# evroon/mav-detection

Measured on NVIDIA B200. Metric: 1080p frame-pairs/sec (flow+FoE+mask), higher is better.
Workload: dtype f32

## Files before the change

mav_detection_b200/csrc/farneback.cu:

```cuda
#include <math.h>

#include "common.cuh"

namespace mavd {

__device__ __forceinline__ int reflect101(int i, int n) {
    while (i < 0 || i >= n) {
        if (n == 1) return 0;
        i = (i < 0) ? -i : 2 * (n - 1) - i;
    }
    return i;
}

__device__ __forceinline__ int clampi(int v, int lo, int hi) { return v < lo ? lo : (v > hi ? hi : v); }

struct PyrLevel {
    int w, h, pitch, taps;
    const int* xbase; const float* xtab;
    const float* xtabT;
    int staged;
    const int* ybase; const float* ytab;
    float* tmp; float* img;
    size_t tmp_stride, img_stride;
    int row0;
// ... 747 lines not shown
            for (int idx = tid; idx < RH * RW; idx += 256) {
                int rr = idx / RW, cc = idx - rr * RW;
                int gy = clampi(y0 - m + rr, 0, h - 1);
                int gx = clampi(x0 - hx + cc, 0, w - 1);
                raw[idx] = __ldg(src + (size_t)gy * pitch + gx);
            }
        }
        __syncthreads();
        const int ncols = IT_TX + 2 * m;
        if (!GAUSS) {
            for (int task = tid; task < ncols * 4; task += 256) {
                int cc = task % ncols + (hx - m), seg = task / ncols;
                const float* col = raw + (seg * 8) * RW + cc;
                float s = 0.f;
                for (int j = 0; j <= 2 * m; ++j) s += col[j * RW];
                float* dst = vs + (seg * 8) * RW + cc;
                dst[0] = s;
#pragma unroll
                for (int o = 1; o < 8; ++o) {
                    s += col[(o + 2 * m) * RW] - col[(o - 1) * RW];
                    dst[o * RW] = s;
                }
            }
        } else {
            for (int task = tid; task < ncols * IT_TY; task += 256) {
                int cc = task % ncols + (hx - m), r = task / ncols;
                const float* col = raw + r * RW + cc;
                float s = __fmul_rn(col[m * RW], __ldg(a.gk));
                for (int i = 1; i <= m; ++i) s = __fmaf_rn(col[(m - i) * RW] + col[(m + i) * RW], __ldg(a.gk + i), s);
                vs[r * RW + cc] = s;
            }
        }
        __syncthreads();
        float* Sc = S + c * (IT_TY * IT_TX);
        if (hx == 8 && m >= 5) {
            for (int task = tid; task < IT_TY * (IT_TX / 4); task += 256) {
                int q = task & 15, r = task >> 4;
                const float4* pv = reinterpret_cast<const float4*>(vs + r * RW + 4 * q);
                float u[20];
#pragma unroll
                for (int j = 0; j < 5; ++j) {
                    float4 v = pv[j];
                    u[4 * j] = v.x; u[4 * j + 1] = v.y; u[4 * j + 2] = v.z; u[4 * j + 3] = v.w;
                }
                float o[4];
                if (!GAUSS) {
                    switch (m) {
                        case 5: hsum_box<5>(u, o); break;
                        case 6: hsum_box<6>(u, o); break;
                        case 7: hsum_box<7>(u, o); break;
                        default: hsum_box<8>(u, o); break;
                    }
                } else {
                    switch (m) {
                        case 5: hsum_gauss<5>(u, a.gk, o); break;
                        case 6: hsum_gauss<6>(u, a.gk, o); break;
                        case 7: hsum_gauss<7>(u, a.gk, o); break;
                        default: hsum_gauss<8>(u, a.gk, o); break;
                    }
                }
                *reinterpret_cast<float4*>(Sc + r * IT_TX + 4 * q) = make_float4(o[0], o[1], o[2], o[3]);
            }
        } else {
            for (int idx = tid; idx < IT_TY * IT_TX; idx += 256) {
                int cx = idx & 63, r = idx >> 6;
                const float* row = vs + r * RW + hx + cx;
                float s;
                if (!GAUSS) {
                    s = 0.f;
                    for (int j = -m; j <= m; ++j) s += row[j];
                } else {
                    s = __fmul_rn(row[0], __ldg(a.gk));
                    for (int i = 1; i <= m; ++i) s = __fmaf_rn(row[-i] + row[i], __ldg(a.gk + i), s);
                }
                Sc[idx] = s;
            }
        }
    }
    __syncthreads();

    const float* R0 = a.R + (size_t)(p * a.pair_stride) * 5 * plane;
    const float* R1 = R0 + 5 * plane;
    float* Mout = LAST ? nullptr : a.Mout + (size_t)p * 5 * plane;
#pragma unroll 2
    for (int j = 0; j < (IT_TX * IT_TY) / 256; ++j) {
        const int idx = j * 256 + tid;
        const int cx = idx & 63, r = idx >> 6;
        const int x = x0 + cx, y = y0 + r;
        if (x >= w || y >= h) continue;
        const float g11 = S[idx] * a.scale, g12 = S[IT_TX * IT_TY + idx] * a.scale,
                    g22 = S[2 * IT_TX * IT_TY + idx] * a.scale, h1 = S[3 * IT_TX * IT_TY + idx] * a.scale,
                    h2 = S[4 * IT_TX * IT_TY + idx] * a.scale;
        const float idet = 1.f / (g11 * g22 - g12 * g12 + 1e-3f);
        const float fx = (g11 * h2 - g12 * h1) * idet;
        const float fy = (g22 * h1 - g12 * h2) * idet;
        if (a.flow) a.flow[(size_t)p * a.flow_stride + (size_t)y * a.flow_pitch + x] = make_float2(fx, fy);
        if (!LAST) update_matrices_px(x, y, w, h, pitch, plane, fx, fy, load_r0_px(R0, (size_t)y * pitch + x, plane), R1, Mout);
    }
}

__device__ __forceinline__ uint32_t smem_u32(const void* p) { return (uint32_t)__cvta_generic_to_shared(p); }

__device__ __forceinline__ void mbar_init(uint64_t* bar, uint32_t count) {
    asm volatile("mbarrier.init.shared::cta.b64 [%0], %1;" ::"r"(smem_u32(bar)), "r"(count));
    asm volatile("fence.mbarrier_init.release.cluster;" ::: "memory");
}
__device__ __forceinline__ void mbar_expect_tx(uint64_t* bar, uint32_t bytes) {
    asm volatile("mbarrier.arrive.expect_tx.shared::cta.b64 _, [%0], %1;" ::"r"(smem_u32(bar)), "r"(bytes) : "memory");
}
__device__ __forceinline__ void mbar_wait(uint64_t* bar, uint32_t parity) {
    asm volatile(
        "{\n"
        ".reg .pred P1;\n"
        "LAB_WAIT:\n"
        "mbarrier.try_wait.parity.shared::cta.b64 P1, [%0], %1;\n"
        "@P1 bra DONE;\n"
        "bra LAB_WAIT;\n"
        "DONE:\n"
        "}" ::"r"(smem_u32(bar)), "r"(parity) : "memory");
}
__device__ __forceinline__ void tma_load_3d(void* dst, const CUtensorMap* map, int c0, int c1, int c2, uint64_t* bar) {
    asm volatile(
        "cp.async.bulk.tensor.3d.shared::cluster.global.mbarrier::complete_tx::bytes [%0], [%1, {%2, %3, %4}], [%5];"
        ::"r"(smem_u32(dst)), "l"(map), "r"(c0), "r"(c1), "r"(c2), "r"(smem_u32(bar)) : "memory");
}

__device__ __forceinline__ void tma_prefetch_3d(const CUtensorMap* map, int c0, int c1, int c2) {
    asm volatile("cp.async.bulk.prefetch.tensor.3d.L2.global.tile [%0, {%1, %2, %3}];"
                 ::"l"(map), "r"(c0), "r"(c1), "r"(c2) : "memory");
}

constexpr int PE_BW = 96;

template <bool U8, int N_>
__global__ void __launch_bounds__(256, 4) polyexp_tma_kernel(const __grid_constant__ CUtensorMap tmap, int w, int h,
                                                         int pitch, PolyConst pc, float* __restrict__ R, size_t plane) {
    pdl_entry();
    __shared__ __align__(128) float raw[(PE_TY + 2 * PE_H) * PE_RW];
    __shared__ __align__(128) float t[3][PE_TY * PE_RW];
    __shared__ __align__(8) uint64_t bar;
    const int tid = threadIdx.x;
    const int x0 = blockIdx.x * PE_TX, y0 = blockIdx.y * PE_TY;
    const int n = N_ > 0 ? N_ : pc.n;
    const int rows = PE_TY + 2 * n;
    uint8_t* bytes = reinterpret_cast<uint8_t*>(&t[0][0]);
    float* raw0 = raw;
    if (tid == 0) {
        mbar_init(&bar, 1);
        if (U8) {
            mbar_expect_tx(&bar, (uint32_t)((rows + 2) * PE_BW));
            tma_load_3d(bytes, &tmap, x0 - 16, y0 - n - 1, blockIdx.z, &bar);
        } else {
            mbar_expect_tx(&bar, (uint32_t)(rows * PE_RW * sizeof(float)));
            tma_load_3d(raw0, &tmap, x0 - PE_H, y0 - n, blockIdx.z, &bar);
        }
    }
    const bool interior = (x0 - PE_H - 1 >= 0) && (x0 + PE_TX + PE_H + 1 <= w) && (y0 - n - 1 >= 0) &&
                          (y0 + PE_TY + n + 1 <= h);
    __syncthreads();
    mbar_wait(&bar, 0);
    if (U8) {
        if (!interior) {
            for (int rr = tid; rr < rows + 2; rr += 256) {
                uint8_t* row = bytes + rr * PE_BW;
                const int bl = -1 - (x0 - 16), br = w - (x0 - 16);
                if (bl >= 0 && bl + 2 < PE_BW) row[bl] = row[bl + 2];
                if (br >= 2 && br < PE_BW) row[br] = row[br - 2];
            }
            __syncthreads();
            for (int cc = tid; cc < PE_BW; cc += 256) {
                const int bt = -1 - (y0 - n - 1), bb = h - (y0 - n - 1);
                if (bt >= 0 && bt + 2 < rows + 2) bytes[bt * PE_BW + cc] = bytes[(bt + 2) * PE_BW + cc];
                if (bb >= 2 && bb < rows + 2) bytes[bb * PE_BW + cc] = bytes[(bb - 2) * PE_BW + cc];
            }
            __syncthreads();
        }
        const int g = tid % 20, seg = tid / 20;
        const int rps = (rows + 11) / 12;
        const int r0 = seg * rps, r1 = min(rows, r0 + rps);
        if (seg < 12 && r0 < r1) {
            const uint32_t* wp = reinterpret_cast<const uint32_t*>(bytes + r0 * PE_BW + 4 * g + 4);
            float hp[4], hc[4], hn[4];
            blur3_words(wp[0], wp[1], wp[2], hp);
            blur3_words(wp[PE_BW / 4], wp[PE_BW / 4 + 1], wp[PE_BW / 4 + 2], hc);
            for (int i = 0; i < r1 - r0; ++i) {
                const uint32_t* q = wp + (i + 2) * (PE_BW / 4);
                blur3_words(q[0], q[1], q[2], hn);
                float4 v;
                v.x = 0.25f * hp[0] + 0.5f * hc[0] + 0.25f * hn[0];
                v.y = 0.25f * hp[1] + 0.5f * hc[1] + 0.25f * hn[1];
                v.z = 0.25f * hp[2] + 0.5f * hc[2] + 0.25f * hn[2];
                v.w = 0.25f * hp[3] + 0.5f * hc[3] + 0.25f * hn[3];
                *reinterpret_cast<float4*>(&raw0[(r0 + i) * PE_RW + 4 * g]) = v;
#pragma unroll
                for (int k = 0; k < 4; ++k) { hp[k] = hc[k]; hc[k] = hn[k]; }
            }
        }
        __syncthreads();
    }
    if (!interior) {
        const int xlo = max(0, PE_H - x0), xhi = min(PE_RW, w - x0 + PE_H);
        const int ylo = max(0, n - y0), yhi = min(rows, h - y0 + n);
        const int ncol = xlo + (PE_RW - xhi);
        if (ncol > 0) {
            for (int idx = tid; idx < (yhi - ylo) * ncol; idx += 256) {
                const int rr = ylo + idx / ncol, k = idx % ncol;
                float* row = raw0 + rr * PE_RW;
                row[k < xlo ? k : xhi + (k - xlo)] = row[k < xlo ? xlo : xhi - 1];
            }
            __syncthreads();
        }
        const int nrow_out = ylo + (rows - yhi);
        if (nrow_out > 0) {
            for (int idx = tid; idx < nrow_out * (PE_RW / 4); idx += 256) {
                const int k = idx / (PE_RW / 4), q = idx - k * (PE_RW / 4);
                const int rr = k < ylo ? k : yhi + (k - ylo);
                reinterpret_cast<float4*>(raw0 + rr * PE_RW)[q] =
                    reinterpret_cast<const float4*>(raw0 + (k < ylo ? ylo : yhi - 1) * PE_RW)[q];
            }
            __syncthreads();
        }
    }
    polyexp_passes<N_>(raw0 - (PE_H - n) * PE_RW, t, pc, n, tid, x0, y0, h, pitch, R + (size_t)blockIdx.z * 5 * plane, plane);
}


__device__ __forceinline__ R0Px load_r0(const float* __restrict__ R0, unsigned o, unsigned plane) {
    R0Px r;
    r.y = __ldg(R0 + o); r.x = __ldg(R0 + (o + plane)); r.yy = __ldg(R0 + (o + 2 * plane));
    r.xx = __ldg(R0 + (o + 3 * plane)); r.xy = __ldg(R0 + (o + 4 * plane));
    return r;
}

template <int RW, int RH>
__device__ __forceinline__ void update_matrices_box(int x, int y, int w, int h, int pitch, unsigned plane, bool edge, float dx,
                                                    float dy, const R0Px& r0, const float* __restrict__ R1,
                                                    float* __restrict__ Mout, const float* box, int bx, int by) {
    constexpr int CH = RH * RW;
    const unsigned o = (unsigned)(y * pitch + x);
    const float r0y = r0.y, r0x = r0.x, r0yy = r0.yy, r0xx = r0.xx, r0xy = r0.xy;
    float fx = (float)x + dx, fy = (float)y + dy;
    const float flx = floorf(fx), fly = floorf(fy);
    const int x1 = (int)fminf(fmaxf(flx, -2.f), 1.0e6f), y1 = (int)fminf(fmaxf(fly, -2.f), 1.0e6f);
    fx -= flx;
    fy -= fly;
    float r2, r3, r4, r5, r6;
    if ((unsigned)x1 < (unsigned)(w - 1) && (unsigned)y1 < (unsigned)(h - 1)) {
        const float gx = 1.f - fx, gy = 1.f - fy;
        const float a00 = gx * gy, a01 = fx * gy, a10 = gx * fy, a11 = fx * fy;
        const int lx = x1 - bx, ly = y1 - by;
        if ((unsigned)lx < (unsigned)(RW - 1) && (unsigned)ly < (unsigned)(RH - 1)) {
            const float* q = box + ly * RW + lx;
            r2 = a00 * q[0] + a01 * q[1] + a10 * q[RW] + a11 * q[RW + 1];
            r3 = a00 * q[CH] + a01 * q[CH + 1] + a10 * q[CH + RW] + a11 * q[CH + RW + 1];
            r4 = a00 * q[2 * CH] + a01 * q[2 * CH + 1] + a10 * q[2 * CH + RW] + a11 * q[2 * CH + RW + 1];
            r5 = a00 * q[3 * CH] + a01 * q[3 * CH + 1] + a10 * q[3 * CH + RW] + a11 * q[3 * CH + RW + 1];
            r6 = a00 * q[4 * CH] + a01 * q[4 * CH + 1] + a10 * q[4 * CH + RW] + a11 * q[4 * CH + RW + 1];
        } else {
            const unsigned q0 = (unsigned)(y1 * pitch + x1), q1 = q0 + (unsigned)pitch;
            r2 = a00 * __ldg(R1 + q0) + a01 * __ldg(R1 + q0 + 1) + a10 * __ldg(R1 + q1) + a11 * __ldg(R1 + q1 + 1);
            r3 = a00 * __ldg(R1 + (q0 + plane)) + a01 * __ldg(R1 + (q0 + plane) + 1) +
                 a10 * __ldg(R1 + (q1 + plane)) + a11 * __ldg(R1 + (q1 + plane) + 1);
            r4 = a00 * __ldg(R1 + (q0 + 2 * plane)) + a01 * __ldg(R1 + (q0 + 2 * plane) + 1) +
                 a10 * __ldg(R1 + (q1 + 2 * plane)) + a11 * __ldg(R1 + (q1 + 2 * plane) + 1);
            r5 = a00 * __ldg(R1 + (q0 + 3 * plane)) + a01 * __ldg(R1 + (q0 + 3 * plane) + 1) +
                 a10 * __ldg(R1 + (q1 + 3 * plane)) + a11 * __ldg(R1 + (q1 + 3 * plane) + 1);
            r6 = a00 * __ldg(R1 + (q0 + 4 * plane)) + a01 * __ldg(R1 + (q0 + 4 * plane) + 1) +
                 a10 * __ldg(R1 + (q1 + 4 * plane)) + a11 * __ldg(R1 + (q1 + 4 * plane) + 1);
        }
        r4 = (r0yy + r4) * 0.5f;
        r5 = (r0xx + r5) * 0.5f;
        r6 = (r0xy + r6) * 0.25f;
    } else {
        r2 = r3 = 0.f;
        r4 = r0yy;
        r5 = r0xx;
        r6 = r0xy * 0.5f;
    }
    r2 = (r0y - r2) * 0.5f;
    r3 = (r0x - r3) * 0.5f;
    r2 += r4 * dy + r6 * dx;
    r3 += r6 * dy + r5 * dx;
    if (edge && ((unsigned)(x - 5) >= (unsigned)(w - 10) || (unsigned)(y - 5) >= (unsigned)(h - 10))) {
        const float sc = (x < 5 ? border_factor(x) : 1.f) * (x >= w - 5 ? border_factor(w - x - 1) : 1.f) *
                         (y < 5 ? border_factor(y) : 1.f) * (y >= h - 5 ? border_factor(h - y - 1) : 1.f);
        r2 *= sc; r3 *= sc; r4 *= sc; r5 *= sc; r6 *= sc;
    }
    st_global_f32(Mout + o, r4 * r4 + r6 * r6);
    st_global_f32(Mout + (o + plane), (r4 + r5) * r6);
    st_global_f32(Mout + (o + 2 * plane), r5 * r5 + r6 * r6);
    st_global_f32(Mout + (o + 3 * plane), r4 * r2 + r6 * r3);
    st_global_f32(Mout + (o + 4 * plane), r6 * r2 + r5 * r3);
}

template <int M_, bool LAST, int TY, bool GAUSS>
__global__ void __launch_bounds__(256, 3) iter_box_tma_kernel(const __grid_constant__ CUtensorMap tmap,
                                                              const __grid_constant__ CUtensorMap tmapR,
                                                              const __grid_constant__ CUtensorMap tmapRbox, IterArgs a) {
    pdl_entry();
    constexpr int NT = 256;
    constexpr int RW = IT_TX + 16;
    constexpr int RH = TY + 2 * M_;
    constexpr int CH = RH * RW;
    constexpr int NC = IT_TX + 2 * M_;
    constexpr int NW = NT / 32;
    extern __shared__ __align__(128) float box[];
    __shared__ __align__(8) uint64_t bar;
    const int tid = threadIdx.x, lane = tid & 31, warp = tid >> 5;
    const int n_tiles = gridDim.x / a.n_pairs;
    int p, tile;
    if (LAST) {
        p = blockIdx.x / n_tiles;
        tile = blockIdx.x - p * n_tiles;
    } else {
        const int per_group = IT_PAIR_GROUP * n_tiles;
        const int gidx = blockIdx.x / per_group, rem = blockIdx.x - gidx * per_group;
        const int gsize = min(IT_PAIR_GROUP, a.n_pairs - gidx * IT_PAIR_GROUP);
        tile = rem / gsize;
        p = gidx * IT_PAIR_GROUP + (rem - tile * gsize);
    }
    const int x0 = (tile % a.tiles_x) * IT_TX, y0 = (tile / a.tiles_x) * TY;
    const int w = a.w, h = a.h, pitch = a.pitch;
    const int plane = (int)a.plane;
    float gk[M_ + 1];
#pragma unroll
    for (int i = 0; i <= M_; ++i) gk[i] = GAUSS ? __ldg(a.gk + i) : 0.f;
    auto hsum = [&](const float (&u)[20], float (&o)[4]) {
        if (GAUSS) hsum_gauss_reg<M_>(u, gk, o);
        else hsum_box<M_>(u, o);
    };

    if (tid == 0) {
        mbar_init(&bar, 1);
        mbar_expect_tx(&bar, 5 * CH * (uint32_t)sizeof(float));
        tma_load_3d(box, &tmap, x0 - 8, y0 - M_, p * 5, &bar);
        if (!LAST) tma_prefetch_3d(&tmapR, x0 - 8, y0 - 8, p * a.pair_stride * 5);
    }
    const bool interior = (x0 - 8 >= 0) && (x0 + IT_TX + 8 <= w) && (y0 - M_ >= 0) && (y0 + TY + M_ <= h);
    __syncthreads();
    mbar_wait(&bar, 0);

    if (!interior) {
        const int xlo = max(0, 8 - x0), xhi = min(RW, w - x0 + 8);
        const int ylo = max(0, M_ - y0), yhi = min(RH, h - y0 + M_);
        const int ncol = xlo + (RW - xhi), nrow_in = yhi - ylo;
        if (ncol > 0) {
            const int per_plane = nrow_in * ncol;
            for (int idx = tid; idx < 5 * per_plane; idx += NT) {
                const int c = idx / per_plane, rem = idx - c * per_plane;
                const int rr = ylo + rem / ncol, k = rem % ncol;
                const int cc = k < xlo ? k : xhi + (k - xlo);
                float* row = box + c * CH + rr * RW;
                row[cc] = row[k < xlo ? xlo : xhi - 1];
            }
            __syncthreads();
        }
        const int nrow_out = ylo + (RH - yhi);
        if (nrow_out > 0) {
            const int per_plane = nrow_out * (RW / 4);
            for (int idx = tid; idx < 5 * per_plane; idx += NT) {
                const int c = idx / per_plane, rem = idx - c * per_plane;
                const int k = rem / (RW / 4), q = rem - k * (RW / 4);
                const int rr = k < ylo ? k : yhi + (k - ylo);
                float* pl = box + c * CH;
                reinterpret_cast<float4*>(pl + rr * RW)[q] = reinterpret_cast<const float4*>(pl + (k < ylo ? ylo : yhi - 1) * RW)[q];
            }
            __syncthreads();
        }
    }

    for (int t = warp; t < 15; t += NW) {
        const int c = t / 3, col = (t - 3 * c) * 32 + lane;
        if (col < NC) {
            float* q = box + c * CH + (8 - M_) + col;
            float in[RH];
            float s = 0.f;
#pragma unroll
            for (int j = 0; j <= 2 * M_; ++j) {
                in[j] = q[j * RW];
                s += in[j];
            }
            if (GAUSS) {
#pragma unroll
                for (int y = 0; y < TY; ++y) {
                    float g = __fmul_rn(in[y + M_], gk[0]);
#pragma unroll
                    for (int i = 1; i <= M_; ++i) g = __fmaf_rn(in[y + M_ - i] + in[y + M_ + i], gk[i], g);
                    q[y * RW] = g;
                    if (y < TY - 1) in[y + 2 * M_ + 1] = q[(y + 2 * M_ + 1) * RW];
                }
                continue;
            }
#pragma unroll
            for (int y = 0; y < TY; ++y) {
                q[y * RW] = s;
                if (y < TY - 1) {
                    in[y + 2 * M_ + 1] = q[(y + 2 * M_ + 1) * RW];
                    if (((y + 1) & 7) == 0) {
                        s = 0.f;
#pragma unroll
                        for (int j = 0; j <= 2 * M_; ++j) s += in[y + 1 + j];
                    } else {
                        s += in[y + 2 * M_ + 1] - in[y];
                    }
                }
            }
        }
    }
    __syncthreads();

    if (LAST) {
        const int q4 = tid & 15, rsub = tid >> 4;
        constexpr int ROWS_PER_IT = NT / 16;
        float2* fl = a.flow + (size_t)p * a.flow_stride;
        const float scale = a.scale;
        const bool vec_ok = (a.flow_pitch & 1) == 0 && (reinterpret_cast<uintptr_t>(fl) & 15) == 0;
#pragma unroll 1
        for (int it = 0; it < TY / ROWS_PER_IT; ++it) {
            const int r = it * ROWS_PER_IT + rsub;
            float o[5][4];
#pragma unroll
            for (int c = 0; c < 5; ++c) {
                const float* row = box + c * CH + r * RW + 4 * q4;
                float u[20];
#pragma unroll
                for (int j = 0; j < 5; ++j) {
                    const float4 v = *reinterpret_cast<const float4*>(row + 4 * j);
                    u[4 * j] = v.x; u[4 * j + 1] = v.y; u[4 * j + 2] = v.z; u[4 * j + 3] = v.w;
                }
                hsum(u, o[c]);
                if (GAUSS) asm volatile("" ::: "memory");
            }
            const int x = x0 + 4 * q4, y = y0 + r;
            if (y >= h || x >= w) continue;
            float2 f[4];
#pragma unroll
            for (int k = 0; k < 4; ++k) {
                const float g11 = o[0][k] * scale, g12 = o[1][k] * scale, g22 = o[2][k] * scale, h1 = o[3][k] * scale,
                            h2 = o[4][k] * scale;
                const float idet = __frcp_rn(g11 * g22 - g12 * g12 + 1e-3f);
                f[k] = make_float2((g11 * h2 - g12 * h1) * idet, (g22 * h1 - g12 * h2) * idet);
            }
            float2* dst = fl + (size_t)y * a.flow_pitch + x;
            if (vec_ok && x + 4 <= w) {
                reinterpret_cast<float4*>(dst)[0] = make_float4(f[0].x, f[0].y, f[1].x, f[1].y);
                reinterpret_cast<float4*>(dst)[1] = make_float4(f[2].x, f[2].y, f[3].x, f[3].y);
            } else {
#pragma unroll
                for (int k = 0; k < 4; ++k)
                    if (x + k < w) dst[k] = f[k];
            }
        }
        return;
    }

    const float* R0 = a.R + (size_t)(p * a.pair_stride) * 5 * a.plane;
    const float* R1 = R0 + 5 * a.plane;
    float* Mout = a.Mout + (size_t)p * 5 * a.plane;
    asm volatile("" : "+l"(Mout));
    const bool edge = (x0 < 5) || (y0 < 5) || (x0 + IT_TX > w - 5) || (y0 + TY > h - 5);
    const float scale = a.scale;
    constexpr int PPT = (IT_TX * TY) / NT;
    __shared__ int s_org[2];
    float ffx[PPT], ffy[PPT];
    {
        static_assert(TY % 16 == 0, "16 rows per pass");
        const int q4 = tid & 15, rsub = tid >> 4;
        constexpr int NPASS = TY / 16;
        float4 gx[NPASS], gy[NPASS];
#pragma unroll
        for (int it = 0; it < NPASS; ++it) {
            const int r = it * 16 + rsub;
            float o[5][4];
#pragma unroll
            for (int c = 0; c < 5; ++c) {
                const float* row = box + c * CH + r * RW + 4 * q4;
                float u[20];
#pragma unroll
                for (int j = 0; j < 5; ++j) {
                    const float4 v = *reinterpret_cast<const float4*>(row + 4 * j);
                    u[4 * j] = v.x; u[4 * j + 1] = v.y; u[4 * j + 2] = v.z; u[4 * j + 3] = v.w;
                }
                hsum(u, o[c]);
            }
            float fx4[4], fy4[4];
#pragma unroll
            for (int k = 0; k < 4; ++k) {
                const float g11 = o[0][k] * scale, g12 = o[1][k] * scale, g22 = o[2][k] * scale,
                            h1 = o[3][k] * scale, h2 = o[4][k] * scale;
                const float idet = __frcp_rn(g11 * g22 - g12 * g12 + 1e-3f);
                fx4[k] = (g11 * h2 - g12 * h1) * idet;
                fy4[k] = (g22 * h1 - g12 * h2) * idet;
            }
            gx[it] = make_float4(fx4[0], fx4[1], fx4[2], fx4[3]);
            gy[it] = make_float4(fy4[0], fy4[1], fy4[2], fy4[3]);
        }
        __syncthreads();
#pragma unroll
        for (int it = 0; it < NPASS; ++it) {
            const int o4 = (it * 16 + rsub) * IT_TX + 4 * q4;
            *reinterpret_cast<float4*>(box + o4) = gx[it];
            *reinterpret_cast<float4*>(box + IT_TX * TY + o4) = gy[it];
        }
        __syncthreads();
    }
#pragma unroll
    for (int j = 0; j < PPT; ++j) {
        const int idx = j * NT + tid;
        const int cx = idx & 63, r = idx >> 6;
        ffx[j] = box[idx];
        ffy[j] = box[IT_TX * TY + idx];
        if (cx == IT_TX / 2 && r == TY / 2) {
            const float cfx = fminf(fmaxf(ffx[j], -1.0e5f), 1.0e5f), cfy = fminf(fmaxf(ffy[j], -1.0e5f), 1.0e5f);
            s_org[0] = ((x0 + (int)floorf(cfx == cfx ? cfx : 0.f)) & ~3) - 8;
            s_org[1] = y0 + (int)floorf(cfy == cfy ? cfy : 0.f) - M_;
        }
    }
    __syncthreads();
    const int bx = s_org[0], by = s_org[1];
    if (tid == 0) {
        asm volatile("fence.proxy.async.shared::cta;" ::: "memory");
        mbar_expect_tx(&bar, 5 * CH * (uint32_t)sizeof(float));
        tma_load_3d(box, &tmapRbox, bx, by, (p * a.pair_stride + 1) * 5, &bar);
    }
    const int cxp = tid & 63, xp = x0 + cxp;
    const bool col_ok = xp < w;
    auto r0_of = [&](int j) {
        const int y = y0 + ((j * NT + tid) >> 6);
        return (col_ok && y < h) ? load_r0(R0, (unsigned)(y * pitch + xp), (unsigned)plane) : R0Px{0.f, 0.f, 0.f, 0.f, 0.f};
    };
    R0Px cur = r0_of(0);
    mbar_wait(&bar, 1);
#pragma unroll
    for (int j = 0; j < PPT; ++j) {
        const int y = y0 + ((j * NT + tid) >> 6);
        R0Px nxt = cur;
        if (j + 1 < PPT) nxt = r0_of(j + 1);
        if (col_ok && y < h)
            update_matrices_box<RW, RH>(xp, y, w, h, pitch, (unsigned)plane, edge, ffx[j], ffy[j], cur, R1, Mout, box, bx, by);
        cur = nxt;
    }
}

__global__ void tap_planar_kernel(const float* __restrict__ src, int w, int h, int pitch, size_t plane, int nch,
                                  float* __restrict__ dst) {
    int x = blockIdx.x * blockDim.x + threadIdx.x, y = blockIdx.y;
    if (x >= w) return;
    for (int c = 0; c < nch; ++c) dst[((size_t)y * w + x) * nch + c] = src[c * plane + (size_t)y * pitch + x];
}
__global__ void tap_flow_kernel(const float2* __restrict__ src, int w, int h, int pitch, float2* __restrict__ dst) {
    int x = blockIdx.x * blockDim.x + threadIdx.x, y = blockIdx.y;
    if (x >= w) return;
    dst[(size_t)y * w + x] = src[(size_t)y * pitch + x];
}

template <bool GAUSS, bool LAST>
static int launch_iter(const IterArgs& a, dim3 grid, size_t smem, cudaStream_t s, bool pdl) {
    MAVD_CUDA((ensure_dynamic_smem<iter_kernel<GAUSS, LAST>>(200 * 1024)));
    MAVD_CUDA(launch_chained(pdl, iter_kernel<GAUSS, LAST>, grid, 256, smem, s, a));
    MAVD_LAUNCHED();
    return MAVD_OK;
}

template <int M_, bool LAST, int TY, bool GAUSS>
static int launch_iter_tma(const CUtensorMap& map, const CUtensorMap& mapR, const CUtensorMap& mapRbox, const IterArgs& a,
                           dim3 grid, cudaStream_t s, bool pdl) {
    constexpr size_t smem = sizeof(float) * 5 * (TY + 2 * M_) * (IT_TX + 16);
    MAVD_CUDA((ensure_dynamic_smem<iter_box_tma_kernel<M_, LAST, TY, GAUSS>>(smem)));
    MAVD_CUDA(launch_chained(pdl, iter_box_tma_kernel<M_, LAST, TY, GAUSS>, grid, 256, smem, s, map, mapR, mapRbox, a));
    MAVD_LAUNCHED();
    return MAVD_OK;
}

template <bool LAST>
static int launch_iter_tma_m(int m, bool gauss, bool small_tiles, const CUtensorMap& map, const CUtensorMap& mapR,
                             const CUtensorMap& mapRbox, const IterArgs& a, dim3 grid, cudaStream_t s, bool pdl) {
    using Launch = int (*)(const CUtensorMap&, const CUtensorMap&, const CUtensorMap&, const IterArgs&, dim3, cudaStream_t,
                           bool);
#define ITER_TMA_M(TY, GAUSS)                                                                                             \
    { launch_iter_tma<5, LAST, TY, GAUSS>, launch_iter_tma<6, LAST, TY, GAUSS>, launch_iter_tma<7, LAST, TY, GAUSS>,     \
      launch_iter_tma<8, LAST, TY, GAUSS> }
    static const Launch table[2][2][4] = {
        {ITER_TMA_M(IT_TY, false), ITER_TMA_M(16, false)},
        {ITER_TMA_M(IT_TY, true), ITER_TMA_M(16, true)}};
#undef ITER_TMA_M
    return table[gauss][small_tiles][m - 5](map, mapR, mapRbox, a, grid, s, pdl);
}

int farneback_run(mavd_handle H, const uint8_t* d_frames, int n_pairs, int pair_stride, float* d_flow,
                  cudaStream_t s) {
    const mavd_farneback_params& fp = H->cfg.farneback;
    const int W = H->cfg.width, Hh = H->cfg.height;
    const int n_frames = pair_stride == 1 ? n_pairs + 1 : 2 * n_pairs;
    const bool gauss = (fp.flags & MAVD_FARNEBACK_GAUSSIAN) != 0;
    const int m = fp.winsize / 2;
    const int hx = round_up(m, 4);
    const size_t frame_bytes = (size_t)W * Hh;

    auto lane = [&](cudaStream_t st) { return (st == H->s_aux && st != s) ? 1 : 0; };
    pdl_break(H, 0);
    pdl_break(H, 1);
    auto build_pyramid = [&](cudaStream_t st, int lo, int hi) -> int {
        if (H->n_levels <= 1 || lo > hi) return MAVD_OK;
        ProfScope ps(&H->prof, MAVD_PROF_PYRAMID, st);
        const int Wp = round_up(W, 4);
        const bool pyr_staged_env = H->tune.pyr_staged != 0;
        const int word_ok = ((W & 3) == 0 && (reinterpret_cast<uintptr_t>(d_frames) & 3) == 0) ? 1 : 0;
        auto make_desc = [&](int a, int b, PyrDesc& d, int& rows) {
            d.n = b - a + 1;
            rows = 0;
            for (int li = a; li <= b; ++li) {
                const Level& L = H->lv[li];
                PyrLevel& P = d.lv[li - a];
                P.w = L.w; P.h = L.h; P.pitch = L.pitch; P.taps = round_up(L.ksz + 1, 4);
                P.xbase = L.xbase; P.xtab = L.xtab; P.ybase = L.ybase; P.ytab = L.ytab;
                P.tmp = L.tmp; P.img = L.img; P.tmp_stride = (size_t)L.h * Wp; P.img_stride = L.plane;
                P.xtabT = L.xtabT;
                P.staged = (pyr_staged_env && L.hspan_max <= PYR_SPAN_MAX && L.hstride_min >= 8) ? 1 : 0;
                P.row0 = rows;
                rows += ceil_div(L.h, 4);
                P.htiles_x = ceil_div(L.w, 64);
            }
        };
        int nv = 0, nh = 0;
        if (H->tune.pyr_sweep != 0 && lo == 1 && word_ok) {
            while (nv < VS_MAXLV && 1 + nv <= hi && H->lv[1 + nv].y_half) ++nv;
            while (nh < HP_MAXLV && 1 + nh <= hi && H->lv[1 + nh].x_half) ++nh;
        }
        MAVD_REQUIRE(n_frames <= 65535, MAVD_ERR_UNSUPPORTED, "pyramid: grid too large");
        if (nv > 0) {
            VSweepDesc vd;
            memset(&vd, 0, sizeof(vd));
            for (int l = 0; l < nv; ++l) {
                const Level& L = H->lv[1 + l];
                vd.tmp[l] = L.tmp; vd.tmp_stride[l] = (size_t)L.h * Wp; vd.h[l] = L.h;
                memcpy(vd.w[l], L.ywt, sizeof(float) * VS_MAXT);
            }
            const int words = W / 4, h_top = H->lv[nv].h;
            int nb = H->tune.pyr_sweep >= 2 ? H->tune.pyr_sweep
                                            : ceil_div(148 * 768, max(1, words * n_frames));
            nb = max(1, min(nb, max(1, h_top / 4)));
            vd.band_rows = ceil_div(h_top, nb);
            nb = ceil_div(h_top, vd.band_rows);
            int tb = 128, waste = 1 << 30;
            for (int cand : {192, 160, 128, 96, 64}) {
                const int wst = ceil_div(words, cand) * cand - words;
                if (wst < waste) { waste = wst; tb = cand; }
            }
            const dim3 g(ceil_div(words, tb), nb, n_frames);
            const bool pdl = pdl_next(H, lane(st));
            const bool h1_fused = nh >= 1;
            if (h1_fused) {
                const Level& L1 = H->lv[1];
                vd.img1 = L1.img; vd.img1_stride = L1.plane; vd.pitch1 = L1.pitch;
                memcpy(vd.xw1, L1.xwt, sizeof(vd.xw1));
            }
#define VS_ARGS g, tb, 0, st, d_frames, frame_bytes, W, Hh, Wp, vd
            switch (nv * 2 + (h1_fused ? 1 : 0)) {
                case 2: MAVD_CUDA(launch_chained(pdl, pyr_vsweep_kernel<1, false>, VS_ARGS)); break;
                case 3: MAVD_CUDA(launch_chained(pdl, pyr_vsweep_kernel<1, true>, VS_ARGS)); break;
                case 4: MAVD_CUDA(launch_chained(pdl, pyr_vsweep_kernel<2, false>, VS_ARGS)); break;
                case 5: MAVD_CUDA(launch_chained(pdl, pyr_vsweep_kernel<2, true>, VS_ARGS)); break;
                case 6: MAVD_CUDA(launch_chained(pdl, pyr_vsweep_kernel<3, false>, VS_ARGS)); break;
                case 7: MAVD_CUDA(launch_chained(pdl, pyr_vsweep_kernel<3, true>, VS_ARGS)); break;
                case 8: MAVD_CUDA(launch_chained(pdl, pyr_vsweep_kernel<4, false>, VS_ARGS)); break;
                default: MAVD_CUDA(launch_chained(pdl, pyr_vsweep_kernel<4, true>, VS_ARGS)); break;
            }
#undef VS_ARGS
            MAVD_LAUNCHED();
        }
        if (lo + nv <= hi) {
            PyrDesc d;
            int rows = 0;
            make_desc(lo + nv, hi, d, rows);
            MAVD_REQUIRE(rows <= 65535, MAVD_ERR_UNSUPPORTED, "pyramid: grid too large");
            MAVD_CUDA(launch_chained(pdl_next(H, lane(st)), pyr_vfirst_kernel, dim3(ceil_div(W, 256), rows, n_frames), 256, 0, st,
                                     d_frames, frame_bytes, W, Hh, Wp, word_ok, d));
            MAVD_LAUNCHED();
        }
        for (int l = nv >= 1 ? 2 : 1; l <= nh; ++l) {
            const Level& L = H->lv[l];
            HPassW hw;
            memcpy(hw.w, L.xwt, sizeof(hw.w));
            const dim3 g(ceil_div(l <= 2 ? ceil_div(L.w, 4) : L.w, 128), L.h, n_frames);
            MAVD_REQUIRE(L.h <= 65535, MAVD_ERR_UNSUPPORTED, "pyramid: grid too large");
            const bool pdl = pdl_next(H, lane(st));
#define HP_ARGS g, 128, 0, st, (const float*)L.tmp, (size_t)L.h * Wp, W, Wp, L.w, L.img, L.plane, L.pitch, hw
            switch (l) {
                case 1: MAVD_CUDA(launch_chained(pdl, pyr_hpass_kernel<1>, HP_ARGS)); break;
                case 2: MAVD_CUDA(launch_chained(pdl, pyr_hpass_kernel<2>, HP_ARGS)); break;
                case 3: MAVD_CUDA(launch_chained(pdl, pyr_hpass1_kernel<3>, HP_ARGS)); break;
                case 4: MAVD_CUDA(launch_chained(pdl, pyr_hpass1_kernel<4>, HP_ARGS)); break;
                case 5: MAVD_CUDA(launch_chained(pdl, pyr_hpass1_kernel<5>, HP_ARGS)); break;
                default: MAVD_CUDA(launch_chained(pdl, pyr_hpass1_kernel<6>, HP_ARGS)); break;
            }
#undef HP_ARGS
            MAVD_LAUNCHED();
        }
        if (lo + nh <= hi) {
            PyrDesc d;
            int rows = 0;
            make_desc(lo + nh, hi, d, rows);
            MAVD_REQUIRE(rows <= 65535, MAVD_ERR_UNSUPPORTED, "pyramid: grid too large");
            for (int a0 = 0; a0 < d.n;) {
                int a1 = a0, hx = 0;
                while (a1 < d.n && d.lv[a1].staged == d.lv[a0].staged) { hx = max(hx, d.lv[a1].htiles_x); ++a1; }
                const int r0 = d.lv[a0].row0, r1 = a1 < d.n ? d.lv[a1].row0 : rows;
                MAVD_CUDA(launch_chained(pdl_next(H, lane(st)), d.lv[a0].staged ? pyr_hsecond_staged_kernel : pyr_hsecond_kernel,
                                         dim3(hx, r1 - r0, n_frames), 256, 0, st, W, Wp, r0, d));
                MAVD_LAUNCHED();
                a0 = a1;
            }
        }
        return MAVD_OK;
    };
    auto expand_level = [&](int li, cudaStream_t st) -> int {
        Level& L = H->lv[li];
        ProfScope ps(&H->prof, MAVD_PROF_POLYEXP, st);
        dim3 g(ceil_div(L.w, PE_TX), ceil_div(L.h, PE_TY), n_frames);
        const int aligned = ((reinterpret_cast<uintptr_t>(d_frames) & 3) == 0 && (W & 3) == 0) ? 1 : 0;
        CUtensorMap tmap_u8;
        bool use_tma = H->tune.polyexp_tma != 0;
        if (use_tma && li == 0)
            use_tma = (W % 16 == 0) && encode_tensor_map_3d(&tmap_u8, true, d_frames, (uint64_t)W, (uint64_t)Hh,
                                                            (uint64_t)n_frames, (uint64_t)W, (uint64_t)W * Hh, PE_BW,
                                                            (uint32_t)(PE_TY + 2 * H->poly.n + 2), 1u);
        else if (use_tma)
            use_tma = L.has_tmap_img;
        const bool pdl = pdl_next(H, lane(st));
#define PE_LAUNCH(N)                                                                                                   \
        do {                                                                                                           \
            if (li == 0 && use_tma)                                                                                    \
                MAVD_CUDA(launch_chained(pdl, polyexp_tma_kernel<true, N>, g, 256, 0, st, tmap_u8, L.w, L.h, L.pitch,   \
                                         H->poly, L.R, L.plane));                                                      \
            else if (li == 0)                                                                                          \
                MAVD_CUDA(launch_chained(pdl, polyexp_kernel<true, N>, g, 256, 0, st, (const void*)d_frames,            \
                                         frame_bytes, L.w, L.h, L.pitch, aligned, H->poly, L.R, L.plane));              \
            else if (use_tma)                                                                                          \
                MAVD_CUDA(launch_chained(pdl, polyexp_tma_kernel<false, N>, g, 256, 0, st, L.tmapImg, L.w, L.h,         \
                                         L.pitch, H->poly, L.R, L.plane));                                             \
            else                                                                                                       \
                MAVD_CUDA(launch_chained(pdl, polyexp_kernel<false, N>, g, 256, 0, st, (const void*)L.img, L.plane,     \
                                         L.w, L.h, L.pitch, 0, H->poly, L.R, L.plane));                                \
        } while (0)
        switch (H->poly.n) {
            case 5: PE_LAUNCH(5); break;
            case 7: PE_LAUNCH(7); break;
            case 8: PE_LAUNCH(8); break;
            default: PE_LAUNCH(0); break;
        }
#undef PE_LAUNCH
        MAVD_LAUNCHED();
        return MAVD_OK;
    };
    auto solve_level = [&](int li, cudaStream_t st) -> int {
        Level& L = H->lv[li];
        {
            ProfScope ps(&H->prof, MAVD_PROF_MATRICES, st);
            const bool top = (li == H->n_levels - 1);
            const Level* C = top ? nullptr : &H->lv[li + 1];
            const bool tables = H->tune.mat_coord == 1, no_pow2 = H->tune.mat_coord == 2;
            const double xscale = top ? 1.0 : 1.0 / ((double)L.w / C->w), yscale = top ? 1.0 : 1.0 / ((double)L.h / C->h);
            auto is_pow2 = [](double v) { int e; return v > 0.0 && frexp(v, &e) == 0.5 && e > -20 && e <= 1; };
            const int coord = tables ? MI_COORD_TABLES
                                     : (!no_pow2 && is_pow2(xscale) && is_pow2(yscale)) ? MI_COORD_POW2 : MI_COORD_F64;
            const dim3 g3(n_pairs, ceil_div(L.w, MI_TX), ceil_div(L.h, MI_TY));
#define MI_ARGS L.R, L.plane, L.w, L.h, L.pitch, (size_t)pair_stride * 5 * L.plane,                                     \
                top ? nullptr : (const float2*)C->flow, top ? 0 : C->w, top ? 0 : C->h, top ? 0 : C->pitch,             \
                top ? 0 : C->plane, L.fxi0, L.fxa, L.fyi0, L.fya, (float)(1.0 / fp.pyr_scale), L.M[0], xscale, yscale, 1
            const bool pdl = pdl_next(H, lane(st));
            if (coord == MI_COORD_TABLES) MAVD_CUDA(launch_chained(pdl, matrices_init_kernel<MI_COORD_TABLES>, g3, 256, 0, st, MI_ARGS));
            else if (coord == MI_COORD_POW2) MAVD_CUDA(launch_chained(pdl, matrices_init_kernel<MI_COORD_POW2>, g3, 256, 0, st, MI_ARGS));
            else MAVD_CUDA(launch_chained(pdl, matrices_init_kernel<MI_COORD_F64>, g3, 256, 0, st, MI_ARGS));
#undef MI_ARGS
            MAVD_LAUNCHED();
        }
        int cur = 0;
        for (int it = 0; it < fp.iterations; ++it) {
            const bool last = (it == fp.iterations - 1);
            IterArgs a;
            a.Min = L.M[cur];
            a.Mout = L.M[cur ^ 1];
            a.R = L.R;
            a.w = L.w; a.h = L.h; a.pitch = L.pitch; a.plane = L.plane;
            a.m = m; a.hx = hx;
            a.scale = gauss ? 1.f : (float)(1.0 / ((double)fp.winsize * fp.winsize));
            a.pair_stride = pair_stride;
            a.gk = gauss ? H->gauss_win : nullptr;
            if (last) {
                if (li == 0) {
                    a.flow = (float2*)d_flow; a.flow_pitch = W; a.flow_stride = (size_t)W * Hh;
                } else {
                    a.flow = (float2*)L.flow; a.flow_pitch = L.pitch; a.flow_stride = L.plane;
                }
            } else {
                a.flow = nullptr; a.flow_pitch = 0; a.flow_stride = 0;
            }
            dim3 g(ceil_div(L.w, IT_TX), ceil_div(L.h, IT_TY), n_pairs);
            a.n_pairs = n_pairs;
            a.tiles_x = g.x;
            const bool small_tiles =
                H->tune.iter_small_tiles != 0 && L.has_tmap16 && (long long)g.x * g.y * g.z <= 3LL * 148;
            const dim3 g1(small_tiles ? g.x * ceil_div(L.h, 16) * g.z : g.x * g.y * g.z);
            const int RW = IT_TX + 2 * hx, RH = IT_TY + 2 * m;
            const size_t smem = sizeof(float) * ((size_t)RH * RW + (size_t)IT_TY * RW + 5 * IT_TX * IT_TY);
            ProfScope ps(&H->prof, li > 0 ? MAVD_PROF_ITER_COARSE : (last ? MAVD_PROF_ITER_FULL_LAST : MAVD_PROF_ITER_FULL), st);
            int rc;
            const bool pdl = pdl_next(H, lane(st));
            if (m >= 5 && m <= 8 && L.has_tmap && !H->force_generic_iter) {
                const CUtensorMap& mM = small_tiles ? L.tmapM16[cur] : L.tmapM[cur];
                const CUtensorMap& mRb = small_tiles ? L.tmapRbox16 : L.tmapRbox;
                rc = last ? launch_iter_tma_m<true>(m, gauss, small_tiles, mM, L.tmapR, mRb, a, g1, st, pdl)
                          : launch_iter_tma_m<false>(m, gauss, small_tiles, mM, L.tmapR, mRb, a, g1, st, pdl);
            }
// ... 84 lines not shown
```

Baseline: 5583.

## Widen horizontal pass to 8 pixels per thread with swizzled rows and prefetch next tile

```diff
diff --git a/mav_detection_b200/csrc/farneback.cu b/mav_detection_b200/csrc/farneback.cu
--- a/mav_detection_b200/csrc/farneback.cu
+++ b/mav_detection_b200/csrc/farneback.cu
@@ -1073,24 +1073,31 @@
     constexpr int RW = IT_TX + 16;
     constexpr int RH = TY + 2 * M_;
     constexpr int CH = RH * RW;
-    constexpr int NC = IT_TX + 2 * M_;
     constexpr int NW = NT / 32;
+    constexpr bool WIDE = TY == 32;
+    constexpr int PX = WIDE ? 8 : 4;
+    constexpr int NPASS = TY * (IT_TX / PX) / NT;
     extern __shared__ __align__(128) float box[];
     __shared__ __align__(8) uint64_t bar;
     const int tid = threadIdx.x, lane = tid & 31, warp = tid >> 5;
     const int n_tiles = gridDim.x / a.n_pairs;
-    int p, tile;
-    if (LAST) {
-        p = blockIdx.x / n_tiles;
-        tile = blockIdx.x - p * n_tiles;
-    } else {
-        const int per_group = IT_PAIR_GROUP * n_tiles;
-        const int gidx = blockIdx.x / per_group, rem = blockIdx.x - gidx * per_group;
-        const int gsize = min(IT_PAIR_GROUP, a.n_pairs - gidx * IT_PAIR_GROUP);
-        tile = rem / gsize;
-        p = gidx * IT_PAIR_GROUP + (rem - tile * gsize);
-    }
-    const int x0 = (tile % a.tiles_x) * IT_TX, y0 = (tile / a.tiles_x) * TY;
+    auto locate = [&](int b, int& p, int& x0, int& y0) {
+        int tile;
+        if (LAST) {
+            p = b / n_tiles;
+            tile = b - p * n_tiles;
+        } else {
+            const int per_group = IT_PAIR_GROUP * n_tiles;
+            const int gidx = b / per_group, rem = b - gidx * per_group;
+            const int gsize = min(IT_PAIR_GROUP, a.n_pairs - gidx * IT_PAIR_GROUP);
+            tile = rem / gsize;
+            p = gidx * IT_PAIR_GROUP + (rem - tile * gsize);
+        }
+        x0 = (tile % a.tiles_x) * IT_TX;
+        y0 = (tile / a.tiles_x) * TY;
+    };
+    int p, x0, y0;
+    locate(blockIdx.x, p, x0, y0);
     const int w = a.w, h = a.h, pitch = a.pitch;
     const int plane = (int)a.plane;
     float gk[M_ + 1];
@@ -1100,12 +1107,60 @@
         if (GAUSS) hsum_gauss_reg<M_>(u, gk, o);
         else hsum_box<M_>(u, o);
     };
+    auto hpos = [&](int it, int& r, int& xo) {
+        if (WIDE) {
+            const int qw = lane >> 3, i = lane & 7;
+            r = 4 * warp + 2 * (qw >> 1) + (i >> 2);
+            xo = 8 * (4 * (qw & 1) + (i & 3));
+        } else {
+            r = it * 16 + (tid >> 4);
+            xo = 4 * (tid & 15);
+        }
+    };
+    auto hrow = [&](int c, int r, int xo, float (&o)[PX]) {
+        const float* row = box + c * CH + r * RW + xo;
+        float u[4 * (PX / 4 + 4)];
+        if (WIDE) {
+            const int sw = (r & 1) * 4;
+            const float* re = row + sw;
+            const float* ro = row - sw;
+#pragma unroll
+            for (int j = 0; j < 6; ++j) {
+                const float4 v = *reinterpret_cast<const float4*>(((j & 1) ? ro : re) + 4 * j);
+                u[4 * j] = v.x; u[4 * j + 1] = v.y; u[4 * j + 2] = v.z; u[4 * j + 3] = v.w;
+            }
+        } else {
+#pragma unroll
+            for (int j = 0; j < 5; ++j) {
+                const float4 v = *reinterpret_cast<const float4*>(row + 4 * j);
+                u[4 * j] = v.x; u[4 * j + 1] = v.y; u[4 * j + 2] = v.z; u[4 * j + 3] = v.w;
+            }
+        }
+#pragma unroll
+        for (int g = 0; g < PX / 4; ++g) {
+            float v[20], s[4];
+#pragma unroll
+            for (int i = 0; i < 20; ++i) v[i] = u[4 * g + i];
+            hsum(v, s);
+#pragma unroll
+            for (int k = 0; k < 4; ++k) o[4 * g + k] = s[k];
+        }
+    };
+    auto fidx = [&](int r, int cx) { return r * IT_TX + (WIDE ? cx ^ ((r & 1) << 2) : cx); };
 
     if (tid == 0) {
         mbar_init(&bar, 1);
         mbar_expect_tx(&bar, 5 * CH * (uint32_t)sizeof(float));
         tma_load_3d(box, &tmap, x0 - 8, y0 - M_, p * 5, &bar);
         if (!LAST) tma_prefetch_3d(&tmapR, x0 - 8, y0 - 8, p * a.pair_stride * 5);
+        unsigned nsm;
+        asm("mov.u32 %0, %%nsmid;" : "=r"(nsm));
+        const int nb = blockIdx.x + 3 * (int)nsm;
+        if (nb < (int)gridDim.x) {
+            int pn, xn, yn;
+            locate(nb, pn, xn, yn);
+            tma_prefetch_3d(&tmap, xn - 8, yn - M_, pn * 5);
+        }
     }
     const bool interior = (x0 - 8 >= 0) && (x0 + IT_TX + 8 <= w) && (y0 - M_ >= 0) && (y0 + TY + M_ <= h);
     __syncthreads();
@@ -1142,8 +1197,9 @@
 
     for (int t = warp; t < 15; t += NW) {
         const int c = t / 3, col = (t - 3 * c) * 32 + lane;
-        if (col < NC) {
-            float* q = box + c * CH + (8 - M_) + col;
+        if (col < RW) {
+            float* q = box + c * CH + col;
+            float* qo = box + c * CH + (WIDE ? col ^ 4 : col);
             float in[RH];
             float s = 0.f;
 #pragma unroll
@@ -1157,14 +1213,14 @@
                     float g = __fmul_rn(in[y + M_], gk[0]);
 #pragma unroll
                     for (int i = 1; i <= M_; ++i) g = __fmaf_rn(in[y + M_ - i] + in[y + M_ + i], gk[i], g);
-                    q[y * RW] = g;
+                    ((y & 1) ? qo : q)[y * RW] = g;
                     if (y < TY - 1) in[y + 2 * M_ + 1] = q[(y + 2 * M_ + 1) * RW];
                 }
                 continue;
             }
 #pragma unroll
             for (int y = 0; y < TY; ++y) {
-                q[y * RW] = s;
+                ((y & 1) ? qo : q)[y * RW] = s;
                 if (y < TY - 1) {
                     in[y + 2 * M_ + 1] = q[(y + 2 * M_ + 1) * RW];
                     if (((y + 1) & 7) == 0) {
@@ -1181,45 +1237,43 @@
     __syncthreads();
 
     if (LAST) {
-        const int q4 = tid & 15, rsub = tid >> 4;
-        constexpr int ROWS_PER_IT = NT / 16;
         float2* fl = a.flow + (size_t)p * a.flow_stride;
         const float scale = a.scale;
         const bool vec_ok = (a.flow_pitch & 1) == 0 && (reinterpret_cast<uintptr_t>(fl) & 15) == 0;
 #pragma unroll 1
-        for (int it = 0; it < TY / ROWS_PER_IT; ++it) {
-            const int r = it * ROWS_PER_IT + rsub;
-            float o[5][4];
+        for (int it = 0; it < NPASS; ++it) {
+            int r, xo;
+            hpos(it, r, xo);
+            float o[5][PX];
 #pragma unroll
             for (int c = 0; c < 5; ++c) {
-                const float* row = box + c * CH + r * RW + 4 * q4;
-                float u[20];
-#pragma unroll
-                for (int j = 0; j < 5; ++j) {
-                    const float4 v = *reinterpret_cast<const float4*>(row + 4 * j);
-                    u[4 * j] = v.x; u[4 * j + 1] = v.y; u[4 * j + 2] = v.z; u[4 * j + 3] = v.w;
+                hrow(c, r, xo, o[c]);
+                if (GAUSS) asm volatile("" ::: "memory");
+            }
+            const int y = y0 + r;
+            if (y >= h) continue;
+#pragma unroll
+            for (int g = 0; g < PX / 4; ++g) {
+                const int x = x0 + xo + 4 * g;
+                if (x >= w) continue;
+                float2 f[4];
+#pragma unroll
+                for (int k = 0; k < 4; ++k) {
+                    const float g11 = o[0][4 * g + k] * scale, g12 = o[1][4 * g + k] * scale,
+                                g22 = o[2][4 * g + k] * scale, h1 = o[3][4 * g + k] * scale,
+                                h2 = o[4][4 * g + k] * scale;
+                    const float idet = __frcp_rn(g11 * g22 - g12 * g12 + 1e-3f);
+                    f[k] = make_float2((g11 * h2 - g12 * h1) * idet, (g22 * h1 - g12 * h2) * idet);
                 }
-                hsum(u, o[c]);
-                if (GAUSS) asm volatile("" ::: "memory");
-            }
-            const int x = x0 + 4 * q4, y = y0 + r;
-            if (y >= h || x >= w) continue;
-            float2 f[4];
-#pragma unroll
-            for (int k = 0; k < 4; ++k) {
-                const float g11 = o[0][k] * scale, g12 = o[1][k] * scale, g22 = o[2][k] * scale, h1 = o[3][k] * scale,
-                            h2 = o[4][k] * scale;
-                const float idet = __frcp_rn(g11 * g22 - g12 * g12 + 1e-3f);
-                f[k] = make_float2((g11 * h2 - g12 * h1) * idet, (g22 * h1 - g12 * h2) * idet);
-            }
-            float2* dst = fl + (size_t)y * a.flow_pitch + x;
-            if (vec_ok && x + 4 <= w) {
-                reinterpret_cast<float4*>(dst)[0] = make_float4(f[0].x, f[0].y, f[1].x, f[1].y);
-                reinterpret_cast<float4*>(dst)[1] = make_float4(f[2].x, f[2].y, f[3].x, f[3].y);
-            } else {
-#pragma unroll
-                for (int k = 0; k < 4; ++k)
-                    if (x + k < w) dst[k] = f[k];
+                float2* dst = fl + (size_t)y * a.flow_pitch + x;
+                if (vec_ok && x + 4 <= w) {
+                    reinterpret_cast<float4*>(dst)[0] = make_float4(f[0].x, f[0].y, f[1].x, f[1].y);
+                    reinterpret_cast<float4*>(dst)[1] = make_float4(f[2].x, f[2].y, f[3].x, f[3].y);
+                } else {
+#pragma unroll
+                    for (int k = 0; k < 4; ++k)
+                        if (x + k < w) dst[k] = f[k];
+                }
             }
         }
         return;
@@ -1235,43 +1289,42 @@
     __shared__ int s_org[2];
     float ffx[PPT], ffy[PPT];
     {
-        static_assert(TY % 16 == 0, "16 rows per pass");
-        const int q4 = tid & 15, rsub = tid >> 4;
-        constexpr int NPASS = TY / 16;
-        float4 gx[NPASS], gy[NPASS];
+        static_assert(NPASS * NT * PX == IT_TX * TY, "the passes cover the tile");
+        float4 gx[NPASS][PX / 4], gy[NPASS][PX / 4];
 #pragma unroll
         for (int it = 0; it < NPASS; ++it) {
-            const int r = it * 16 + rsub;
-            float o[5][4];
-#pragma unroll
-            for (int c = 0; c < 5; ++c) {
-                const float* row = box + c * CH + r * RW + 4 * q4;
-                float u[20];
-#pragma unroll
-                for (int j = 0; j < 5; ++j) {
-                    const float4 v = *reinterpret_cast<const float4*>(row + 4 * j);
-                    u[4 * j] = v.x; u[4 * j + 1] = v.y; u[4 * j + 2] = v.z; u[4 * j + 3] = v.w;
+            int r, xo;
+            hpos(it, r, xo);
+            float o[5][PX];
+#pragma unroll
+            for (int c = 0; c < 5; ++c) hrow(c, r, xo, o[c]);
+#pragma unroll
+            for (int g = 0; g < PX / 4; ++g) {
+                float fx4[4], fy4[4];
+#pragma unroll
+                for (int k = 0; k < 4; ++k) {
+                    const float g11 = o[0][4 * g + k] * scale, g12 = o[1][4 * g + k] * scale,
+                                g22 = o[2][4 * g + k] * scale, h1 = o[3][4 * g + k] * scale,
+                                h2 = o[4][4 * g + k] * scale;
+                    const float idet = __frcp_rn(g11 * g22 - g12 * g12 + 1e-3f);
+                    fx4[k] = (g11 * h2 - g12 * h1) * idet;
+                    fy4[k] = (g22 * h1 - g12 * h2) * idet;
                 }
-                hsum(u, o[c]);
-            }
-            float fx4[4], fy4[4];
-#pragma unroll
-            for (int k = 0; k < 4; ++k) {
-                const float g11 = o[0][k] * scale, g12 = o[1][k] * scale, g22 = o[2][k] * scale,
-                            h1 = o[3][k] * scale, h2 = o[4][k] * scale;
-                const float idet = __frcp_rn(g11 * g22 - g12 * g12 + 1e-3f);
-                fx4[k] = (g11 * h2 - g12 * h1) * idet;
-                fy4[k] = (g22 * h1 - g12 * h2) * idet;
-            }
-            gx[it] = make_float4(fx4[0], fx4[1], fx4[2], fx4[3]);
-            gy[it] = make_float4(fy4[0], fy4[1], fy4[2], fy4[3]);
+                gx[it][g] = make_float4(fx4[0], fx4[1], fx4[2], fx4[3]);
+                gy[it][g] = make_float4(fy4[0], fy4[1], fy4[2], fy4[3]);
+            }
         }
         __syncthreads();
 #pragma unroll
         for (int it = 0; it < NPASS; ++it) {
-            const int o4 = (it * 16 + rsub) * IT_TX + 4 * q4;
-            *reinterpret_cast<float4*>(box + o4) = gx[it];
-            *reinterpret_cast<float4*>(box + IT_TX * TY + o4) = gy[it];
+            int r, xo;
+            hpos(it, r, xo);
+#pragma unroll
+            for (int g = 0; g < PX / 4; ++g) {
+                const int o4 = fidx(r, xo + 4 * g);
+                *reinterpret_cast<float4*>(box + o4) = gx[it][g];
+                *reinterpret_cast<float4*>(box + IT_TX * TY + o4) = gy[it][g];
+            }
         }
         __syncthreads();
     }
@@ -1279,8 +1332,8 @@
     for (int j = 0; j < PPT; ++j) {
         const int idx = j * NT + tid;
         const int cx = idx & 63, r = idx >> 6;
-        ffx[j] = box[idx];
-        ffy[j] = box[IT_TX * TY + idx];
+        ffx[j] = box[fidx(r, cx)];
+        ffy[j] = box[IT_TX * TY + fidx(r, cx)];
         if (cx == IT_TX / 2 && r == TY / 2) {
             const float cfx = fminf(fmaxf(ffx[j], -1.0e5f), 1.0e5f), cfy = fminf(fmaxf(ffy[j], -1.0e5f), 1.0e5f);
             s_org[0] = ((x0 + (int)floorf(cfx == cfx ? cfx : 0.f)) & ~3) - 8;
```

Result: slower. 5484, median of 6 (-1.8%).
